# tirtho109/parallel_AMG

Measured on AMD Instinct MI355X. Metric: V-cycle iters/sec + fine-SpMV HBM GB/s, 3D Poisson 128M dofs at 1/2/4/8 GPU, higher is better.
Workload: dtype f64; 1 GPU; poisson3d 512^3 fp64, SA-AMG V(1,1) weighted-Jacobi, 1 part(s); n=134217728, nnz_fine=937951232, levels=6, max_coarse=1000, parallelism=row-slab partition p1

## Files before the change

parallel_amg_amd/_lib.py:

```python
from __future__ import annotations

import contextlib
import ctypes as C
import os

_HERE = os.path.dirname(os.path.abspath(__file__))
LIB_PATH = os.environ.get("PAMG_LIB") or os.path.join(_HERE, "libpamg.so")

PAMG_OK = 0
ERRORS = {-1: "PAMG_E_ARG", -2: "PAMG_E_HIP", -3: "PAMG_E_RCCL", -4: "PAMG_E_OVERFLOW",
          -5: "PAMG_E_SETUP", -6: "PAMG_E_STATE", -7: "PAMG_E_NOMEM"}


class PamgError(RuntimeError):
    def __init__(self, code, fn, msg):
        super().__init__(f"{fn} -> {ERRORS.get(code, code)}: {msg}")
        self.code = code


vp = C.c_void_p
i32, i64, dbl = C.c_int, C.c_int64, C.c_double
pvp = C.POINTER(C.c_void_p)
pi64 = C.POINTER(C.c_int64)
pdbl = C.POINTER(C.c_double)
# ... 95 lines not shown
}
_RESTYPE = {"pamg_version": C.c_char_p, "pamg_last_error": C.c_char_p}

_lib = None


def lib():
    global _lib
    if _lib is None:
        if not os.path.exists(LIB_PATH):
            raise ImportError(
                f"{LIB_PATH} is missing: build it with `python -c 'import __graft_entry__ as g; g.build()'` "
                "(or `make -C parallel_amg_amd/csrc`). There is no CPU fallback.")
        L = C.CDLL(LIB_PATH)
        for name, args in SIGNATURES.items():
            f = getattr(L, name)
            f.argtypes = args
            f.restype = _RESTYPE.get(name, C.c_int)
        _lib = L
    return _lib


class _DlInfo(C.Structure):
    _fields_ = [("dli_fname", C.c_char_p), ("dli_fbase", C.c_void_p),
                ("dli_sname", C.c_char_p), ("dli_saddr", C.c_void_p)]


def runtime_providers() -> dict:
    L = lib()
    dl = C.CDLL(None)
    dladdr = dl.dladdr
    dladdr.argtypes = [C.c_void_p, C.POINTER(_DlInfo)]
    out = {}
    for key, sym in (("hip", "hipStreamCreateWithFlags"), ("rccl", "ncclCommInitRank")):
        try:
            addr = C.cast(getattr(L, sym), C.c_void_p).value
        except AttributeError:
            continue
        info = _DlInfo()
        if addr and dladdr(addr, C.byref(info)) and info.dli_fname:
            out[key] = os.path.realpath(info.dli_fname.decode())
    return out


def call(name, *args):
    L = lib()
    rc = getattr(L, name)(*args)
    if rc != PAMG_OK:
        msg = L.pamg_last_error().decode(errors="replace")
        raise PamgError(rc, name, msg)
    return rc


@contextlib.contextmanager
def option(key: str, value: int):
    old = C.c_int64()
    call("pamg_get_option", key.encode(), C.byref(old))
    call("pamg_set_option", key.encode(), int(value))
    try:
        yield
    finally:
        call("pamg_set_option", key.encode(), old.value)


def layout_of(M, part_set: int = 0) -> dict:
    out = (C.c_int * 10)()
    call("pamg_mat_layout", M.handle, part_set, out)
    win = (C.c_int * 16)()
    if part_set == 0:
        call("pamg_mat_ell_window", M.handle, win)
    return {"ell_xwin": bool(win[0]), "ell_xwin_groups": int(win[1]), "ell_gather_groups": int(win[2]),
            "ell_xwin_max_window": int(win[3]), "ell_xwin_noncontig_groups": int(win[4]),
            "ell_xwin_max_pairs": int(win[5]), "ell_xwin_max_chunks": int(win[6]),
            "ell_xwin_census": {"groups": int(win[7]), "full_groups": int(win[13]), "window_mean": int(win[8]),
                                "window_p95": int(win[9]), "runs_mean": int(win[10]), "runs_max": int(win[11]),
                                "pairs_mean": int(win[12])},
            "c24": bool(out[0]), "vd": bool(out[1]), "rl8": bool(out[2]), "cd": int(out[3]),
            "cd_offsets": int(out[4]), "tm": bool(out[5]), "tm_rs": int(out[6]),
            "tile_nnz": int(out[7]), "tiles": int(out[8]), "anchored": bool(out[9] & 1), "per_tile": bool(out[9] & 2),
            "x_stage": bool(out[9] & 4), "sym": bool(out[9] & 8), "sym_rows": 2 if out[9] & 16 else 1,
            "jr_fused": bool(out[9] & 32), "tm_vd": bool(out[9] & 64), "sym_vd": bool(out[9] & 128),
            "ell": bool(out[9] & 512), "pnc": bool(out[9] & 1024),
            "rpat": bool(out[9] & 2048), "pnc_compact": bool(out[9] & 4096),
            "ell_pair": bool(out[9] & 8192)}


def last_error() -> str:
    return lib().pamg_last_error().decode(errors="replace")


def ptr(a):
    return C.c_void_p(a.ctypes.data) if a is not None and a.size else None
```

parallel_amg_amd/csrc/kernels.hip:

```cpp

#include "pamg_device.h"
#include "div_rn.h"

namespace pamg {
namespace {

__device__ __forceinline__ int wave_incl_scan(int v) {
    const int lane = threadIdx.x & 63, rl = lane & 15;
    int t;
    t = __builtin_amdgcn_mov_dpp(v, 0x111, 0xf, 0xf, false);
    if (rl >= 1) v += t;
    t = __builtin_amdgcn_mov_dpp(v, 0x112, 0xf, 0xf, false);
    if (rl >= 2) v += t;
    t = __builtin_amdgcn_mov_dpp(v, 0x114, 0xf, 0xf, false);
    if (rl >= 4) v += t;
    t = __builtin_amdgcn_mov_dpp(v, 0x118, 0xf, 0xf, false);
    if (rl >= 8) v += t;
    t = __builtin_amdgcn_mov_dpp(v, 0x142, 0xf, 0xf, false);
    if (lane & 16) v += t;
    t = __builtin_amdgcn_mov_dpp(v, 0x143, 0xf, 0xf, false);
    if (lane >= 32) v += t;
    return v;
}

// ... 1786 lines not shown
#pragma unroll
    for (int q = 0; q < NS; ++q) {
        zs[q] = zc0 + q * part;
        ze[q] = min(zc1, zs[q] + part);
        zl[q] = ze[q] > zs[q] ? ze[q] - 1 : zc1 - 1;
    }
    PncRow cur[NS];
    int am[NS], ap[NS];
#pragma unroll
    for (int q = 0; q < NS; ++q) {
        const int z = min(zs[q], zl[q]);
        pnc_load<OP, CP>(cur[q], z * M + ixy, nrows, nx, anc, rec, cid, x, b, y);
        am[q] = anc[z > 0 ? (z - 1) * M + ixy : ixy];
        ap[q] = anc[z + 1 < nz ? (z + 1) * M + ixy : ixy];
    }
    __syncthreads();
    for (int j = 0; j < part; ++j) {
        int zq[NS], L[NS], col[NS][kPncMaxLen];
        double xv[NS][kPncMaxLen];
#pragma unroll
        for (int q = 0; q < NS; ++q) {
            zq[q] = min(zs[q] + j, zl[q]);
            const uint32_t pid = CP ? cur[q].rec.x : cur[q].rec.x & 1023u;
            const uint32_t pw = pid < (uint32_t)npat ? lp[pid] : 0u;
            L[q] = (int)(pw & 7u);
#pragma unroll
            for (int k = 0; k < kPncMaxLen; ++k) {
                const uint32_t c = (pw >> (3 + 3 * k)) & 7u;
                const int c01 = c & 1u ? cur[q].an[1] : cur[q].an[0];
                const int c23 = c & 1u ? cur[q].an[3] : cur[q].an[2];
                const int c45 = c & 1u ? am[q] : cur[q].an[4];
                const int c03 = c & 2u ? c23 : c01;
                const int c47 = c & 2u ? ap[q] : c45;
                col[q][k] = c & 4u ? c47 : c03;
                xv[q][k] = x[k < L[q] ? col[q][k] : col[q][0]];
            }
        }
        PncRow nxt[NS];
        int ap2[NS];
#pragma unroll
        for (int q = 0; q < NS; ++q) {
            const int zn = min(zq[q] + 1, zl[q]);
            pnc_load<OP, CP>(nxt[q], zn * M + ixy, nrows, nx, anc, rec, cid, x, b, y);
            ap2[q] = anc[zn + 1 < nz ? (zn + 1) * M + ixy : zn * M + ixy];
        }
#pragma unroll
        for (int q = 0; q < NS; ++q) {
            const int i = zq[q] * M + ixy;
            uint64_t rr;
            if constexpr (CP) rr = cur[q].rec.x < (uint32_t)npat ? lw[cur[q].rec.x] : 0ull;
            else rr = (((uint64_t)cur[q].rec.y << 32) | cur[q].rec.x) >> 10;
            double s = 0.0, dg = 0.0;
#pragma unroll
            for (int k = 0; k < kPncMaxLen; ++k) {
                const bool ok = k < L[q];
                const double v = lv[(uint32_t)(rr >> (7 * k)) & 127u];
                const double p = v * xv[q][k];
                const double t = s + p;
                s = ok ? t : s;
                if constexpr (OP == OP_JACOBI) dg = ok && col[q][k] == i ? v : dg;
            }
            double out;
            if constexpr (OP == OP_SPMV) {
                out = s;
            } else if constexpr (OP == OP_RESID) {
                out = cur[q].p0 - s;
            } else if constexpr (OP == OP_JACOBI) {
                const double uu = cur[q].p0 - s;
                const double v = omega * uu;
                const double w = v / dg;
                out = cur[q].p1 + w;
            } else {
                out = cur[q].p0 + s;
            }
            const bool in = CP ? cur[q].rec.x != (uint32_t)kPncCombSkip : (cur[q].rec.x & 1023u) != (uint32_t)kPncSkip;
            if (zs[q] + j < ze[q] && in) y[i] = out;
            am[q] = cur[q].an[0];
            cur[q] = nxt[q];
            ap[q] = ap2[q];
        }
    }
}

template <int OP>
__global__ __launch_bounds__(kBlock) void k_rows_long(
    const int* __restrict__ rows, const int* __restrict__ rowptr, const int* __restrict__ col,
    const double* __restrict__ val, const double* __restrict__ x, const double* __restrict__ b,
    double* __restrict__ y, double omega, double c1 = 0.0, const double* __restrict__ xold = nullptr) {
    __shared__ double lprod[kBlock + 8];
    __shared__ double ldiag;
    const int tid = threadIdx.x;
    const int r = rows[blockIdx.x];
    const int z0 = rowptr[r], z1 = rowptr[r + 1];
    double s = 0.0;
    for (int base = z0; base < z1; base += kBlock) {
        const int k = base + tid;
        double p = 0.0;
        if (k < z1) {
            const int c = col[k];
            const double v = val[k];
            p = v * x[c];
            if constexpr (kDiagOp<OP>) {
                if (c == r) ldiag = v;
            }
        }
        lprod[tid] = p;
        __syncthreads();
        if (tid == 0) s = row_sum_lds(lprod, 0, min(kBlock, z1 - base), s);
        __syncthreads();
    }
    if constexpr (OP == OP_CHEB) {
        if (tid == 0) epilogue<OP>(r, s, x, b, y, omega, ldiag, c1, xold);
    } else {
        if (tid == 0) epilogue<OP>(r, s, x, b, y, omega, OP == OP_JACOBI ? ldiag : 0.0);
    }
}

__global__ __launch_bounds__(kBlock) void k_cheb_update(int64_t n, const uint8_t* __restrict__ mask, int mask_bytes,
                                                        const uint8_t* __restrict__ ids,
                                                        const uint32_t* __restrict__ mtab, uint32_t in_flag,
                                                        const double* __restrict__ diag, const double* __restrict__ x,
                                                        const double* __restrict__ xold, double* __restrict__ y,
                                                        double c1, double c2) {
    for (int64_t i = blockIdx.x * (int64_t)kBlock + threadIdx.x; i < n; i += (int64_t)gridDim.x * kBlock) {
        const uint32_t m = ids ? mtab[ids[i]]
                               : (mask_bytes == 1 ? (uint32_t)mask[i] : (uint32_t)reinterpret_cast<const uint16_t*>(mask)[i]);
        if (!(m & in_flag)) continue;
        y[i] = cheb_step(y[i], x[i], xold ? xold[i] : 0.0, diag[i], c1, c2);
    }
}

__global__ void k_jacobi_zero(int64_t n, const double* __restrict__ b,
                              const double* __restrict__ diag, double omega,
                              double* __restrict__ y) {
    for (int64_t i = blockIdx.x * (int64_t)blockDim.x + threadIdx.x; i < n;
         i += (int64_t)gridDim.x * blockDim.x) {
        const double u = b[i] - 0.0;
        const double v = omega * u;
        const double w = v / diag[i];
        y[i] = 0.0 + w;
    }
}

constexpr int kGemvChunk = 1024;
__global__ __launch_bounds__(kBlock) void k_dense_gemv(int64_t n_rows, int64_t n,
                                                       int64_t row0,
                                                       const double* __restrict__ ainv,
                                                       const double* __restrict__ b,
                                                       double* __restrict__ y) {
    __shared__ __attribute__((aligned(16))) double lp_all[kBlock / 64][kGemvChunk + 8];
    const int w = threadIdx.x >> 6, lane = threadIdx.x & 63;
    const int64_t i = (int64_t)blockIdx.x * (kBlock / 64) + w;
    if (i >= n_rows) return;
    const double* a = ainv + (row0 + i) * n;
    double* lp = lp_all[w];
    double s = 0.0;
    for (int64_t c = 0; c < n; c += kGemvChunk) {
        const int m = (int)((n - c) < kGemvChunk ? (n - c) : kGemvChunk);
#pragma unroll
        for (int q = 0; q < kGemvChunk / 64; ++q) {
            const int j = lane + 64 * q;
            if (j < m) {
                const double p = a[c + j] * b[c + j];
                lp[j] = p;
            }
        }
// ... 226 lines not shown
          (int64_t)sd.nbands * sd.band >= A.nrows && A.nrows == (int64_t)sd.tb.nx * sd.tb.ny * sd.tb.nz &&
          A.nrows % 2 == 0))
        return false;
    TbGeom g = sd.tb;
    const int tiles = g.tiles_x * g.tiles_y;
    int zc = options().zm_chunks > 0 ? options().zm_chunks : std::min((1024 + tiles - 1) / tiles, g.nz / 16);
    zc = std::max(1, std::min(zc, g.nz));
    g.zlen = (g.nz + zc - 1) / zc;
    g.zchunks = (g.nz + g.zlen - 1) / g.zlen;
    const int gr = (tiles * g.zchunks + 7) / 8 * 8;
    k_sym_zm<OP><<<gr, kZmThreads, 0, s>>>((int)A.nrows, sd.d_tid, sd.d_vtab, sd.d_mtab, sd.vd_n, g, x, b, y, omega,
                                           ch.c1, ch.xold);
    return true;
}

template <int OP, int NU>
void launch_sym_nu(const pamg_mat& A, const double* x, const double* b, double* y, double omega, hipStream_t s) {
    const SymDia& sd = A.sym;
    const int grid = sd.nbands * 8 * sd.eighth;
    if constexpr (NU == 3) {
        if (launch_sym_zm<OP>(A, x, b, y, omega, s)) return;
    }
    if (sd.vd_n) {
        const int ch = NU <= 3 ? options().symd_chunks : 1;
        const int g = 8 * ((sd.nbands * sd.eighth + ch - 1) / ch);
        if constexpr (NU <= 3) {
            if (ch == 2) {
                k_rows_symd<OP, NU, 2><<<g, kBlock, 0, s>>>((int)A.nrows, (int)A.nrows, sd.d_tid, sd.d_vtab,
                                                            sd.d_mtab, sd.vd_n, sd, x, b, y, omega);
                return;
            }
            if (ch == 4) {
                k_rows_symd<OP, NU, 4><<<g, kBlock, 0, s>>>((int)A.nrows, (int)A.nrows, sd.d_tid, sd.d_vtab,
                                                            sd.d_mtab, sd.vd_n, sd, x, b, y, omega);
                return;
            }
        }
        k_rows_symd<OP, NU><<<grid, kBlock, 0, s>>>((int)A.nrows, (int)A.nrows, sd.d_tid, sd.d_vtab, sd.d_mtab,
                                                  sd.vd_n, sd, x, b, y, omega);
        return;
    }
    if (sd.rpl == 2) {
        k_rows_sym2<OP, NU><<<grid, kBlock, 0, s>>>((int)A.nrows, (int)A.nrows, sd.d_mask, sd.d_diag, sd.d_upper,
                                                  sd.ld, sd, x, b, y, omega);
        return;
    }
    k_rows_sym<OP, NU><<<grid, kBlock, 0, s>>>((int)A.nrows, (int)A.nrows, sd.d_mask, sd.d_diag, sd.d_upper, sd.ld,
                                             sd, x, b, y, omega);
}

template <int OP>
void launch_sym(const pamg_mat& A, const double* x, const double* b, double* y, double omega, hipStream_t s,
                Cheb ch = Cheb{}) {
    if constexpr (OP == OP_PROLONG) {
        return;
    } else if constexpr (OP == OP_CHEB) {
        if (launch_sym_zm<OP_CHEB>(A, x, b, y, omega, s, ch)) return;
        launch_sym<OP_RESID>(A, x, b, y, 0.0, s);
        launch_cheb_update(A, x, ch.xold, y, ch.c1, omega, s);
    } else {
        switch (A.sym.nu) {
            case 1: launch_sym_nu<OP, 1>(A, x, b, y, omega, s); break;
            case 2: launch_sym_nu<OP, 2>(A, x, b, y, omega, s); break;
            case 3: launch_sym_nu<OP, 3>(A, x, b, y, omega, s); break;
            case 4: launch_sym_nu<OP, 4>(A, x, b, y, omega, s); break;
            case 5: launch_sym_nu<OP, 5>(A, x, b, y, omega, s); break;
            case 6: launch_sym_nu<OP, 6>(A, x, b, y, omega, s); break;
            default: launch_sym_nu<OP, 7>(A, x, b, y, omega, s); break;
        }
    }
}

constexpr int kPncZlen = 32, kPncStreams = 2;

template <int OP>
void launch_pnc(const pamg_mat& A, const double* x, const double* b, double* y, double omega, hipStream_t s) {
    const PncSet& P = A.pnc;
    const int zlen = std::min(kPncZlen, P.nz);
    const int nxb = P.nx * P.ny / 256, units = nxb * ((P.nz + zlen - 1) / zlen);
    auto go = [&](auto kern) {
        kern<<<(units + 7) / 8 * 8, 256, 0, s>>>((int)A.nrows, P.nx, P.nx * P.ny, P.nz, zlen, P.d_anc, P.d_rec, P.d_cid,
                                                P.d_pvals, P.d_ptab, P.npat, P.d_vtab, P.nval, x, b, y, omega);
    };
    if (P.d_cid) go(k_rows_pnc<OP, kPncStreams, true>);
    else go(k_rows_pnc<OP, kPncStreams, false>);
}

template <int OP>
void launch_rpat(const pamg_mat& A, const double* x, const double* b, double* y, double omega, hipStream_t s) {
    const RpatSet& R = A.rpat;
    const int grid = (int)((R.ngroups + 7) / 8 * 8);
    auto go = [&](auto kern) {
        kern<<<grid, kEllGroup, 0, s>>>((int)A.nrows, R.d_gorder, R.d_anc, R.d_pid, R.d_pmeta, R.npat, R.d_pent, R.nent,
                                        R.d_vtab, R.nval, (int)R.ngroups, x, b, y, omega);
    };
    go(k_rows_rpat<OP, 8>);
}

template <int OP>
void launch_rows_op(const pamg_mat& A, const TileSet& ts, const double* x, const double* b,
                    double* y, double omega, hipStream_t s, Cheb ch = Cheb{}) {
    if (ts.sym) launch_sym<OP>(A, x, b, y, omega, s, ch);
    if (ts.ell) {
        const EllSet& E = A.ell;
        const int grid = (int)((E.ngroups + 7) / 8 * 8);
        auto go = [&](auto kern) {
            kern<<<grid, kEllGroup, 0, s>>>((int)A.nrows, E.d_gorder, E.d_anc, E.d_smeta, E.d_ci, E.d_vi, E.d_len,
                                            E.d_gmeta, E.d_otab, E.d_vtab, (int)E.ngroups, x, b, y, omega, ch.c1,
                                            ch.xold);
        };
        if (E.win) {
            const int win = std::max(E.max_window, 128);
            const size_t lds = sizeof(double) * (size_t)(win + 256) + sizeof(uint16_t) * 4 * 256;
            k_rows_ellw<OP><<<grid, kEllGroup, lds, s>>>(
                (int)A.nrows, E.d_gslices, E.d_smeta, E.d_ci, E.d_len, E.d_dpos, E.d_gmeta, E.d_otab, E.d_vtab, E.d_wmeta,
                E.d_chunks, E.d_lof, win, (reinterpret_cast<uintptr_t>(x) & 15) != 0 ? 1 : 0, (int)E.ngroups, x, b, y,
                omega, ch.c1, ch.xold);
        } else if (E.d_anc) {
            if (E.paired) go(k_rows_ell<OP, true, true>);
            else go(k_rows_ell<OP, true, false>);
        } else {
            if (E.paired) go(k_rows_ell<OP, false, true>);
            else go(k_rows_ell<OP, false, false>);
        }
    }
    if constexpr (OP != OP_CHEB) {
        if (ts.pnc) launch_pnc<OP>(A, x, b, y, omega, s);
        if (ts.rpat) launch_rpat<OP>(A, x, b, y, omega, s);
    }
    if (ts.n_short > 0) {
        if (ts.tile_nnz == 1024) launch_tile<OP, 1024>(A, ts, x, b, y, omega, s, ch);
        else if (ts.tile_nnz == 4096) launch_tile<OP, 4096>(A, ts, x, b, y, omega, s, ch);
        else launch_tile<OP, 2048>(A, ts, x, b, y, omega, s, ch);
    }
    if (ts.n_long > 0)
        k_rows_long<OP><<<ts.n_long, kBlock, 0, s>>>(ts.d_long, A.d_rowptr, A.d_col, A.d_val, x,
                                                     b, y, omega, ch.c1, ch.xold);
}
}

void launch_sym_tb(const pamg_mat& A, const TbArgs& ta, hipStream_t s) {
    SymDia sd = A.sym;
    TbGeom& g = sd.tb;
    g.zlo = sd.part_lo == 0 ? 0 : sd.part_lo + ta.nstages - 1;
    g.zhi = sd.part_hi == g.nz ? g.nz : sd.part_hi - (ta.nstages - 1);
    const int span = g.zhi - g.zlo;
    if (span <= 0) return;
    g.zchunks = std::max(1, std::min(g.zchunks, span / 2 > 0 ? span / 2 : 1));
    g.zlen = (span + g.zchunks - 1) / g.zchunks;
    g.zchunks = (span + g.zlen - 1) / g.zlen;
    const int ntiles = g.tiles_x * g.tiles_y * g.zchunks;
    const int grid = (ntiles + 7) / 8 * 8;
    g.xfast = options().tb_xfast;
    if (sd.vd_n) {
        if (ta.nstages == 2)
            k_sym_zc<2, 2><<<grid, ZcShape<2>::threads, 0, s>>>((int)A.nrows, sd.d_tid, sd.d_vtab, sd.d_mtab, sd.vd_n,
                                                                sd, ta);
        else
            k_sym_zc<3, 1><<<grid, ZcShape<3>::threads, 0, s>>>((int)A.nrows, sd.d_tid, sd.d_vtab, sd.d_mtab, sd.vd_n,
                                                                sd, ta);
        return;
    }
    if (ta.nstages == 2)
        k_sym_tb<2><<<grid, TbShape<2>::threads, 0, s>>>((int)A.nrows, sd.d_mask, sd.d_diag, sd.d_upper, sd.ld, sd, ta);
    else
        k_sym_tb<3><<<grid, TbShape<3>::threads, 0, s>>>((int)A.nrows, sd.d_mask, sd.d_diag, sd.d_upper, sd.ld, sd, ta);
}

// ... 91 lines not shown
```

parallel_amg_amd/csrc/pamg_device.h:

```cpp
#pragma once

#include <hip/hip_runtime.h>
#include <rccl/rccl.h>

#include <atomic>
#include <cstdint>
#include <array>
#include <mutex>
#include <vector>

#include "pamg_common.h"

namespace pamg {

constexpr int kBlock = 256;
constexpr int kTileRows = 256;

constexpr int kXsMaxClusters = 12;
constexpr int kTmSmallTab = 128;
constexpr int kXsCap = 1088;
constexpr int kXsIoff = 128;
constexpr int kXsGap = 48;
struct XStage {
    int ncl = 0, stride = 0, zix = -1, ncols = 0;
// ... 51 lines not shown
    int tile_order = 1;
    int col24 = 1;
    int long_tiles = 1;
    int long_tiles_min = 24;
    int row_len8 = 1;
    int value_dict = 1;
    int col_dict = 1;
    int tile_major = 1;
    int col_dict_tile = 1;
    int tm_tile_dicts = 1;
    int band_pct = 100;
    int band_pct_restrict = 50;
    int x_stage = 1;
    int col_dict_anchor = 1;
    int poison_ghosts = 0;
    int sym_dia = 1;
    int sym_rows = 2;
    int jr_fuse = 1;
    int symd_chunks = 2;
    int chain_store_x = 0;
    int tb_xfast = 1;
    int sym_zm = 1;
    int zm_chunks = 0;
    int ell = 1;
    int ell_min_rows = 65536;
    int ell_restrict = 1;
    int ell_yblock = 16;
    int rpat = 1;
    int ell_pair = 1;
    int ell_xwin = 1;
    int ell_xwin_max = 7168;
    int pnc_compact = 1;
    int pnc = 1;
    int sym_vd = 1;
};

constexpr int kSymMaxU = 7;
constexpr int kSymVdMax = 64;
struct TbGeom {
    int nx = 0, ny = 0, nz = 0;
    int tiles_x = 0, tiles_y = 0;
    int zchunks = 1, zlen = 0;
    int zlo = 0, zhi = 0;
    int xfast = 0;
};
constexpr int kEllW = 64;
constexpr int kEllGroup = 256;
constexpr int kEllSkip = 255;
constexpr int kEllWinCap = 7168;
constexpr int kEllWinChunks = 256;
constexpr int kEllLdsPerCu = 160 * 1024;
constexpr int kEllWinKeep = 85;
constexpr int kEllWinMinShare = 50;
constexpr int kEllWinMinRatio100 = 150;
struct EllSet {
    int64_t nslices = 0, ngroups = 0;
    int2* d_smeta = nullptr;
    uint32_t* d_ci = nullptr;
    uint32_t* d_vi = nullptr;
    uint8_t* d_len = nullptr;
    int4* d_gmeta = nullptr;
    int* d_otab = nullptr;
    double* d_vtab = nullptr;
    int* d_anc = nullptr;
    int* d_gorder = nullptr;
    int64_t words = 0, otab_n = 0, vtab_n = 0;
    bool paired = false;
    bool win = false;
    int4* d_gslices = nullptr;
    int4* d_wmeta = nullptr;
    int2* d_chunks = nullptr;
    uint16_t* d_lof = nullptr;
    uint8_t* d_dpos = nullptr;
    int64_t nchunks = 0, lof_n = 0;
    int win_groups = 0, gather_groups = 0, noncontig_groups = 0;
    int max_window = 0, max_pairs = 0, max_chunks = 0;
    int mean_window = 0, p95_window = 0, mean_runs = 0, max_runs = 0, mean_pairs = 0, full_groups = 0;
};

constexpr int kPncPatMax = 1024, kPncValMax = 128, kPncMaxLen = 7;
constexpr int kPncSkip = kPncPatMax - 1;
constexpr int kPncCombMax = 1024;
constexpr int kPncCombSkip = 0xffff;
struct PncSet {
    int nx = 0, ny = 0, nz = 0;
    int* d_anc = nullptr;
    uint2* d_rec = nullptr;
    uint16_t* d_cid = nullptr;
    uint64_t* d_pvals = nullptr;
    uint32_t* d_ptab = nullptr;
    double* d_vtab = nullptr;
    int npat = 0, nval = 0;
    int grid = 0;
};

constexpr int kRpatMax = 255, kRpatEnt = 4096, kRpatMaxLen = 128;
constexpr int kRpatSkip = 255;
struct RpatSet {
    int64_t ngroups = 0;
    int* d_anc = nullptr;
    uint8_t* d_pid = nullptr;
    int2* d_pmeta = nullptr;
    uint32_t* d_pent = nullptr;
    double* d_vtab = nullptr;
    int* d_gorder = nullptr;
    int npat = 0, nent = 0, nval = 0;
};

struct SymDia {
    int nu = 0;
    int off[kSymMaxU] = {};
    int64_t ld = 0;
    int band = 0, band_blocks = 0, eighth = 0, nbands = 0;
    int rpl = 1;
    bool tb_ok = false;
    bool tb_part = false;
    int part_lo = 0, part_hi = 0;
    int plane0 = 0;
    int gap_at = 1 << 30, gap = 0;
    TbGeom tb;
    uint8_t* d_mask = nullptr;
    int mask_bytes = 2;
    double* d_diag = nullptr;
    double* d_upper = nullptr;
    int vd_n = 0;
    int vd_main = 0;
    uint8_t* d_tid = nullptr;
    double* d_vtab = nullptr;
    uint32_t* d_mtab = nullptr;
};
Options& options();

}

struct pamg_ctx {
    int device = 0;
    std::atomic<int> refs{1};
    hipStream_t s_comp = nullptr;
    hipStream_t s_comm = nullptr;
    hipEvent_t ev_fork = nullptr, ev_join = nullptr;
    ncclComm_t comm = nullptr;
    int rank = 0, nranks = 1;
    pamg_host_comm_fn host_fn = nullptr;
    void* host_user = nullptr;
    pamg_world* world = nullptr;
    hipEvent_t ev_ready = nullptr;
    std::vector<double> h_send, h_recv;
    double* d_red = nullptr;
    int red_cap = 0;
    double* h_red = nullptr;
    char* stage[2] = {nullptr, nullptr};
    hipEvent_t stage_done[2] = {nullptr, nullptr};
    std::vector<std::array<int64_t, 4>> grids;
    std::mutex grids_mu;
};

void ctx_ref(pamg_ctx* ctx);
void ctx_unref(pamg_ctx* ctx);

struct pamg_plan {
    pamg_ctx* ctx = nullptr;
    int64_t n_own = 0, n_ghost = 0;
    std::vector<int> nbr;
    std::vector<int64_t> recv_off, send_off;
    int* d_send_idx = nullptr;
    double* d_sendbuf = nullptr;
// ... 70 lines not shown
```

parallel_amg_amd/csrc/runtime.hip:

```cpp
#include <dlfcn.h>

#include <algorithm>
#include <array>
#include <atomic>
#include <functional>
#include <iterator>
#include <chrono>
#include <cmath>
#include <condition_variable>
#include <mutex>
#include <cstdio>
#include <cstdlib>
#include <cstring>
#include <map>
#include <memory>
#include <mutex>
#include <string>
#include <thread>
#include <vector>

#include "pamg_device.h"

using pamg::fail;

// ... 2068 lines not shown
        (n_own_cols == nrows || pamg::options().ell_restrict)) {
        CHECK(build_ell(A, u.rp, u.ci, u.val, n_own_cols != nrows, u.inner));
        if (A->interior.ell) u.inner.clear();
        u.tr.mark("ell");
    }
    return PAMG_OK;
}

int64_t ell_bytes(const pamg_mat* A) {
    if (!A->interior.ell) return 0;
    const int64_t nrows = A->nrows;
    return (A->ell.paired ? 4 : 8) * A->ell.words + nrows + 8 * A->ell.nslices + 16 * A->ell.ngroups + 4 * A->ell.otab_n +
           8 * A->ell.vtab_n + (A->ell.d_anc ? 4 * nrows : 0) +
           (A->ell.win ? 32 * A->ell.ngroups + 8 * A->ell.nchunks + 2 * A->ell.lof_n + nrows : 0);
}

void ell_report(const pamg_mat* A, const pamg::TileSet& t, int out[10]) {
    if (!t.ell) return;
    out[8] = (int)A->ell.ngroups;
    out[9] |= 512 | (A->ell.paired ? 8192 : 0);
}

void ell_window(const pamg_mat* A, int out[16]) {
    const pamg::EllSet& E = A->ell;
    const bool w = A->interior.ell && E.win;
    out[0] = w ? 1 : 0;
    out[1] = w ? E.win_groups : 0;
    out[2] = w ? E.gather_groups : 0;
    out[3] = w ? E.max_window : 0;
    out[4] = w ? E.noncontig_groups : 0;
    out[5] = w ? E.max_pairs : 0;
    out[6] = w ? E.max_chunks : 0;
    out[7] = w ? (int)E.ngroups : 0;
    out[8] = w ? E.mean_window : 0;
    out[9] = w ? E.p95_window : 0;
    out[10] = w ? E.mean_runs : 0;
    out[11] = w ? E.max_runs : 0;
    out[12] = w ? E.mean_pairs : 0;
    out[13] = w ? E.full_groups : 0;
    out[14] = out[15] = 0;
}

void ell_free(pamg::EllSet& E) {
    dfree(E.d_gorder);
    dfree(E.d_smeta);
    dfree(E.d_ci);
    dfree(E.d_vi);
    dfree(E.d_len);
    dfree(E.d_gmeta);
    dfree(E.d_otab);
    dfree(E.d_vtab);
    dfree(E.d_anc);
    dfree(E.d_gslices);
    dfree(E.d_wmeta);
    dfree(E.d_chunks);
    dfree(E.d_lof);
    dfree(E.d_dpos);
    E = pamg::EllSet{};
}

int pnc_try(Upload& u) {
    pamg_mat* A = u.A;
    const int64_t nrows = A->nrows;
    if (pamg::options().pnc && u.n_own_cols < nrows && (int64_t)u.inner.size() * 4 >= (int64_t)nrows * 3) {
        const auto grids = grids_of(A->ctx);
        for (auto g = grids.rbegin(); g != grids.rend() && !A->interior.pnc; ++g)
            if ((*g)[0] == nrows) CHECK(build_pnc(A, u.rp, u.ci, u.val, *g, u.inner));
        if (A->interior.pnc) u.inner.clear();
        u.tr.mark("pnc");
    }
    return PAMG_OK;
}

int64_t pnc_bytes(const pamg_mat* A) {
    if (!A->interior.pnc) return 0;
    return (A->pnc.d_cid ? 6 : 12) * A->nrows + (A->pnc.d_cid ? 12 : 4) * A->pnc.npat + 8 * A->pnc.nval;
}

void pnc_report(const pamg_mat* A, const pamg::TileSet& t, int out[10]) {
    if (!t.pnc) return;
    out[3] = A->pnc.nval;
    out[4] = A->pnc.npat;
    out[8] = A->pnc.grid;
    out[9] |= 1024 | (A->pnc.d_cid ? 4096 : 0);
}

void pnc_free(pamg::PncSet& P) {
    dfree(P.d_anc);
    dfree(P.d_rec);
    dfree(P.d_cid);
    dfree(P.d_pvals);
    dfree(P.d_ptab);
    dfree(P.d_vtab);
    P = pamg::PncSet{};
}

int tiles_try(Upload& u) {
    pamg_mat* A = u.A;
    pamg_ctx* ctx = A->ctx;
    const PtrVec& rp = u.rp;
    const IdxVec& ci = u.ci;
    const int64_t nrows = A->nrows, nnz = A->nnz, n_own_cols = u.n_own_cols;
    std::vector<uint16_t> lo;
    std::vector<uint8_t> hi, vidx;
    {
        std::vector<int4> t_in, t_bd;
        const bool square = n_own_cols == nrows;
        const bool tall = n_own_cols < nrows;
        const int64_t tb = u.inner.empty() && u.bnd.empty() ? 0 : u.band();
        CHECK(build_tiles(rp, u.inner, square, &A->interior, tb, ci, &lo, &hi, u.val, &vidx, &t_in, tall));
        CHECK(build_tiles(rp, u.bnd, square, &A->boundary, tb, ci, &lo, &hi, u.val, &vidx, &t_bd, tall));
        u.tr.mark("tiles");
        std::vector<uint8_t> idx8;
        CHECK(build_col_dicts(A, rp, ci, t_in, t_bd, &idx8));
        u.tr.mark("col dicts");
        CHECK(build_tile_major(A, n_own_cols, rp, ci, u.val, t_in, t_bd, lo, hi, idx8));
        u.tr.mark("tile-major");
    }
    if (A->interior.rl8 || A->boundary.rl8) {
        std::vector<uint8_t> rl(nrows + kVecPad, 0);
        par_for(nrows, [&](int64_t a, int64_t b) {
            for (int64_t i = a; i < b; ++i) rl[i] = (uint8_t)std::min<int64_t>(255, rp[i + 1] - rp[i]);
        });
        CHECK(dalloc(&A->d_rlen, nrows + kVecPad));
        CHECK(h2d(ctx, A->d_rlen, rl.data(), rl.size()));
    }
    if (!vidx.empty()) {
        CHECK(dalloc(&A->d_vidx, (int64_t)vidx.size()));
        CHECK(h2d(ctx, A->d_vidx, vidx.data(), vidx.size()));
    }
    if (!lo.empty()) {
        lo.resize(nnz + kVecPad, 0);
        hi.resize(nnz + kVecPad, 0);
        CHECK(dalloc(&A->d_clo, nnz + kVecPad));
        CHECK(dalloc(&A->d_chi, nnz + kVecPad));
        CHECK(h2d(ctx, A->d_clo, lo.data(), sizeof(uint16_t) * lo.size()));
        CHECK(h2d(ctx, A->d_chi, hi.data(), sizeof(uint8_t) * hi.size()));
    }
    u.tr.mark("rest");
    return PAMG_OK;
}

int64_t tiles_bytes(const pamg_mat* A) {
    int64_t sum = 0;
    for (const pamg::TileSet* t : {&A->interior, &A->boundary}) {
        if (t->sym || t->ell || t->pnc || t->rpat) continue;
        const int64_t ns = t->n_short, nz = t->nnz_short;
        int64_t b = 8 * (int64_t)t->n_long + 12 * t->nnz_long;
        const bool base = t->c24 && !t->cd;
        if (t->tm) {
            const int64_t tn = t->tile_nnz;
            const int64_t rowb = t->tm_rs;
            const int64_t valb = t->tm_vt ? tn + 8 * (int64_t)t->tm_vt : 8 * tn;
            b += ns * (rowb * (t->anc ? 5 : 1) + valb + (t->cd ? t->cd * tn / 8 : 3 * tn) + 16 + (base ? 4 : 0)) +
                 (t->cd ? 4 * t->ctab_n * (t->pt ? ns : 1) : 0);
        } else {
            b += (t->rl8 ? 1 : 4) * t->rows_short;
            b += t->cd ? (t->cd * nz + 7) / 8 + 4 * t->ctab_n * (t->pt ? ns : 1) : (t->c24 ? 3 : 4) * nz;
            if (t->pt && t->anc) b += 2 * t->rows_short + 4 * ns;
            b += t->vd ? nz / 2 + 128 * ns : 8 * nz;
            b += (16 + (base ? 4 : 0)) * ns;
        }
        sum += b;
    }
    return sum;
}

// ... 2090 lines not shown
        CHECK(dalloc(&H->pcg_p, cap));
        CHECK(dalloc(&H->pcg_q, cap));
        for (double* p : {H->pcg_r, H->pcg_z, H->pcg_p, H->pcg_q})
            CHECK(dzero(ctx, p, sizeof(double) * cap));
    }
    hipStream_t s = ctx->s_comp;
    double *r = H->pcg_r, *z = H->pcg_z, *p = H->pcg_p, *q = H->pcg_q;
    DeviceSpace d(H, x, b, true);
    double* xd = d.x;
    CHECK(apply(ctx, A, pamg::OP_RESID, xd, d.b, r, 0.0));
    double rr = 0.0;
    CHECK(reduce_scalar(ctx, n, r, r, &rr));
    const double nr0 = std::sqrt(rr);
    if (res_hist) res_hist[0] = nr0;
    int k = 0;
    if (nr0 > 0.0 && maxit > 0) {
        CHECK(vcycle_raw(H, z, r, 1, true));
        HIPC(hipMemcpyAsync(p, z, sizeof(double) * n, hipMemcpyDeviceToDevice, s));
        double rz = 0.0;
        CHECK(reduce_scalar(ctx, n, r, z, &rz));
        while (k < maxit) {
            ++k;
            CHECK(apply(ctx, A, pamg::OP_SPMV, p, nullptr, q, 0.0));
            double pq = 0.0;
            CHECK(reduce_scalar(ctx, n, p, q, &pq));
            const double alpha = rz / pq;
            CHECK(reduce_with(ctx, n, &rr, [&](int np, double* parts, double* res, hipStream_t st) {
                pamg::launch_cg_update(n, alpha, p, q, xd, r, parts, np, res, st);
            }));
            const double nr = std::sqrt(rr);
            if (res_hist) res_hist[k] = nr;
            if (nr <= rtol * nr0) break;
            CHECK(vcycle_raw(H, z, r, 1, true));
            double rz_new = 0.0;
            CHECK(reduce_scalar(ctx, n, r, z, &rz_new));
            const double beta = rz_new / rz;
            rz = rz_new;
            pamg::launch_axpby(n, 1.0, z, beta, p, s);
        }
    }
    d.finish(x);
    HIPC(hipGetLastError());
    HIPC(hipStreamSynchronize(s));
    if (iters) *iters = k;
    return PAMG_OK;
}

}

namespace {
struct OptionRow {
    const char* key;
    int pamg::Options::*member;
    int64_t lo, hi;
    bool pow2;
};
using O = pamg::Options;
const OptionRow kOptionTable[] = {
    {"tile_nnz", &O::tile_nnz, 1024, 4096, true},
    {"tile_order", &O::tile_order, 0, 1, false},
    {"poison_ghosts", &O::poison_ghosts, 0, 1, false},
    {"col24", &O::col24, 0, 1, false},
    {"long_tiles", &O::long_tiles, 0, 1, false},
    {"row_len8", &O::row_len8, 0, 1, false},
    {"value_dict", &O::value_dict, 0, 2, false},
    {"col_dict", &O::col_dict, 0, 1, false},
    {"tile_major", &O::tile_major, 0, 2, false},
    {"col_dict_anchor", &O::col_dict_anchor, 0, 1, false},
    {"col_dict_tile", &O::col_dict_tile, 0, 1, false},
    {"x_stage", &O::x_stage, 0, 1, false},
    {"band_pct", &O::band_pct, 1, 10000, false},
    {"band_pct_restrict", &O::band_pct_restrict, 1, 10000, false},
    {"long_tiles_min", &O::long_tiles_min, 1, 255, false},
    {"tm_tile_dicts", &O::tm_tile_dicts, 0, 1, false},
    {"sym_dia", &O::sym_dia, 0, 1, false},
    {"sym_rows", &O::sym_rows, 1, 2, false},
    {"jr_fuse", &O::jr_fuse, 0, 1, false},
    {"sym_vd", &O::sym_vd, 0, 1, false},
    {"symd_chunks", &O::symd_chunks, 1, 4, true},
    {"sym_zm", &O::sym_zm, 0, 1, false},
    {"tb_xfast", &O::tb_xfast, 0, 1, false},
    {"ell", &O::ell, 0, 1, false},
    {"ell_restrict", &O::ell_restrict, 0, 1, false},
    {"pnc", &O::pnc, 0, 1, false},
    {"rpat", &O::rpat, 0, 1, false},
    {"pnc_compact", &O::pnc_compact, 0, 1, false},
    {"ell_pair", &O::ell_pair, 0, 1, false},
    {"ell_xwin", &O::ell_xwin, 0, 1, false},
    {"ell_xwin_max", &O::ell_xwin_max, 2, pamg::kEllWinCap, false},
    {"ell_yblock", &O::ell_yblock, 0, 65536, false},
    {"ell_min_rows", &O::ell_min_rows, 0, INT32_MAX, false},
    {"zm_chunks", &O::zm_chunks, 0, 4096, false},
    {"chain_store_x", &O::chain_store_x, 0, 1, false},
};

const OptionRow* find_option(const char* key) {
    for (const OptionRow& r : kOptionTable)
        if (std::strcmp(r.key, key) == 0) return &r;
    return nullptr;
}
}

extern "C" {

int pamg_set_option(const char* key, int64_t value) {
    if (!key) return fail(PAMG_E_ARG, "set_option: NULL key");
    const OptionRow* r = find_option(key);
    if (!r || value < r->lo || value > r->hi || (r->pow2 && (value & (value - 1)) != 0))
        return fail(PAMG_E_ARG, "set_option: unknown key or bad value: %s=%lld", key, (long long)value);
    pamg::options().*(r->member) = (int)value;
    return PAMG_OK;
}

int pamg_get_option(const char* key, int64_t* value) {
    if (!key || !value) return fail(PAMG_E_ARG, "get_option: bad args");
    const OptionRow* r = find_option(key);
    if (!r) return fail(PAMG_E_ARG, "get_option: unknown key %s", key);
    *value = pamg::options().*(r->member);
    return PAMG_OK;
}

int pamg_hier_bench_chain(pamg_hier* H, pamg_vec* x, const pamg_vec* b, int reps, double* avg_ms) {
    if (!H || !x || !b || reps < 1 || !avg_ms) return fail(PAMG_E_ARG, "hier_bench_chain: bad args");
    if (!pipe_ok(H, 2, false)) return fail(PAMG_E_STATE, "hier_bench_chain: the hierarchy does not run the cross-cycle pipeline");
    pamg_ctx* ctx = H->ctx;
    CHECK(check_vec_for(H->A[0], x, "hier_bench_chain"));
    CHECK(set_device(ctx));
    CHECK(ensure_u0(H));
    int k = -1;
    return time_reps(ctx->s_comp, reps, avg_ms, [&]() {
        const bool back = k > 0 && (k & 1);
        ++k;
        return launch_chain3(H, x->d, b->d, back ? H->u0 : H->t[0], back ? H->t[0] : H->u0);
    });
}

int pamg_bench_rowop(pamg_ctx* ctx, const pamg_mat* A, int op, pamg_vec* x, const pamg_vec* b,
                     pamg_vec* y, double omega, int reps, double* avg_ms) {
    if (!ctx || !A || !x || !y || reps < 1 || !avg_ms || op < 0 || op > 6)
        return fail(PAMG_E_ARG, "bench_rowop: bad args");
    if ((op == pamg::OP_RESID || op == pamg::OP_JACOBI || op >= 4) && !b) return fail(PAMG_E_ARG, "bench_rowop: b needed");
    if ((op == pamg::OP_JACOBI || op >= 4) && !A->d_diag)
        return fail(PAMG_E_SETUP, "bench_rowop: jacobi needs a square matrix");
    if (op == pamg::OP_CHEB) {
        if (A->interior.pnc || A->interior.rpat) return fail(PAMG_E_ARG, "bench_rowop: op 6 needs a square operator");
        if (x == y || b == y) return fail(PAMG_E_ARG, "bench_rowop: y must differ from x and b");
        CHECK(check_vec_for(A, x, "bench_rowop"));
        if (b->n_own != A->nrows || y->n_own != A->nrows) return fail(PAMG_E_ARG, "bench_rowop: size mismatch");
        CHECK(set_device(ctx));
        double* xo = nullptr;
        CHECK(dalloc(&xo, A->nrows + kVecPad));
        int rc = dzero(ctx, xo, sizeof(double) * (size_t)(A->nrows + kVecPad));
        hipStream_t s = ctx->s_comp;
        if (rc == PAMG_OK)
            rc = time_reps(s, reps, avg_ms, [&]() {
                pamg::launch_rows(*A, A->interior, op, x->d, b->d, xo, y->d, omega, s, omega);
                pamg::launch_rows(*A, A->boundary, op, x->d, b->d, xo, y->d, omega, s, omega);
                return PAMG_OK;
            });
        dfree(xo);
        return rc;
    }
    if (op >= 4 && !(A->interior.sym && (A->sym.tb_ok || A->sym.tb_part)))
        return fail(PAMG_E_STATE, "bench_rowop: op %d needs the temporally blocked layout (pamg_mat_layout bit 5)", op);
    if (op == pamg::OP_PROLONG && (A->interior.sym || A->boundary.sym))
        return fail(PAMG_E_STATE, "bench_rowop: the symmetric layouts have no prolongate-add kernel");
    if (x == y) return fail(PAMG_E_ARG, "bench_rowop: x and y must differ");
// ... 42 lines not shown
```

Measured before the change: 225.2 V-cycles/s.

## Add 2D-tiled pattern-compressed row kernel sharing anchor indices through LDS

Adds a new pattern-compressed (pnc) row kernel that processes a 64x4 xy tile per block and marches along z. Each lane's anchor column indices for its x/y neighbours come from a double-buffered LDS plane with a halo ring, and z-neighbour anchors are carried in registers. This replaces per-row anchor reads from global memory with shared reuse. It is selected when the pnc option is 1 and the grid dims divide the tile, and the option range is widened to 2 so the old kernel stays reachable. The cost is extra LDS, one block barrier per z step, and higher register pressure.

```diff
diff --git a/parallel_amg_amd/_lib.py b/parallel_amg_amd/_lib.py
--- a/parallel_amg_amd/_lib.py
+++ b/parallel_amg_amd/_lib.py
@@ -201,7 +201,7 @@
             "jr_fused": bool(out[9] & 32), "tm_vd": bool(out[9] & 64), "sym_vd": bool(out[9] & 128),
             "ell": bool(out[9] & 512), "pnc": bool(out[9] & 1024),
             "rpat": bool(out[9] & 2048), "pnc_compact": bool(out[9] & 4096),
-            "ell_pair": bool(out[9] & 8192)}
+            "ell_pair": bool(out[9] & 8192), "pnc_tiled": bool(out[9] & 16384)}
 
 
 def last_error() -> str:
diff --git a/parallel_amg_amd/csrc/kernels.hip b/parallel_amg_amd/csrc/kernels.hip
--- a/parallel_amg_amd/csrc/kernels.hip
+++ b/parallel_amg_amd/csrc/kernels.hip
@@ -1892,6 +1892,196 @@
     }
 }
 
+struct PnctRow {
+    uint2 rec;
+    double p0, p1;
+    int am, a0, ap;
+    int rg;
+};
+
+template <int OP, int NS, bool CP, int TX, int TY>
+__global__ __launch_bounds__(256) void k_rows_pnct(int nrows, int nx, int M, int nz, int zlen,
+                                                   const int* __restrict__ anc, const uint2* __restrict__ rec,
+                                                   const uint16_t* __restrict__ cid, const uint64_t* __restrict__ pvals,
+                                                   const uint32_t* __restrict__ ptab, int npat,
+                                                   const double* __restrict__ vtab, int nval,
+                                                   const double* __restrict__ x, const double* __restrict__ b,
+                                                   double* __restrict__ y, double omega) {
+    static_assert(TX * TY == 256 && 2 * TX + 2 * TY <= 256, "one row per lane; one ring point per edge thread");
+    constexpr int LW = TX + 2, LP = LW * (TY + 2);
+    __shared__ uint32_t lp[CP ? kPncCombMax : kPncPatMax];
+    __shared__ uint64_t lw[CP ? kPncCombMax : 1];
+    __shared__ double lv[kPncValMax];
+    __shared__ int la[NS][2][LP];
+    const int nxb = M >> 8;
+    const int units = nxb * ((nz + zlen - 1) / zlen);
+    const int per = (units + 7) >> 3;
+    const int u = (int)(blockIdx.x & 7) * per + (int)(blockIdx.x >> 3);
+    if (u >= units) return;
+    const int tid = (int)threadIdx.x;
+    for (int t = tid; t < npat; t += 256) lp[t] = ptab[t];
+    if constexpr (CP)
+        for (int t = tid; t < npat; t += 256) lw[t] = pvals[t];
+    for (int t = tid; t < nval; t += 256) lv[t] = vtab[t];
+    const int zc0 = (u / nxb) * zlen, zc1 = min(nz, zc0 + zlen);
+    const int part = (zc1 - zc0 + NS - 1) / NS;
+    const int tpx = nx / TX, ny = M / nx, tb = u % nxb;
+    const int x0 = (tb % tpx) * TX, y0 = (tb / tpx) * TY;
+    const int ixy = (y0 + tid / TX) * nx + x0 + tid % TX;
+    const int lpos = (tid / TX + 1) * LW + tid % TX + 1;
+    int rxy = -1, rpos = 0;
+    if (tid < TX) {
+        rxy = (y0 > 0 ? y0 - 1 : y0) * nx + x0 + tid;
+        rpos = tid + 1;
+    } else if (tid < 2 * TX) {
+        rxy = (y0 + TY < ny ? y0 + TY : y0 + TY - 1) * nx + x0 + tid - TX;
+        rpos = (TY + 1) * LW + tid - TX + 1;
+    } else if (tid >= 256 - TY) {
+        rxy = (y0 + tid - (256 - TY)) * nx + (x0 + TX < nx ? x0 + TX : x0 + TX - 1);
+        rpos = (tid - (256 - TY) + 1) * LW + TX + 1;
+    } else if (tid >= 256 - 2 * TY) {
+        rxy = (y0 + tid - (256 - 2 * TY)) * nx + (x0 > 0 ? x0 - 1 : x0);
+        rpos = (tid - (256 - 2 * TY) + 1) * LW;
+    }
+    int zs[NS], ze[NS], zl[NS], za[NS];
+    PnctRow r[NS];
+#pragma unroll
+    for (int q = 0; q < NS; ++q) {
+        zs[q] = zc0 + q * part;
+        ze[q] = min(zc1, zs[q] + part);
+        zl[q] = ze[q] > zs[q] ? ze[q] - 1 : zc1 - 1;
+        const int z = za[q] = min(zs[q], zl[q]), zp = min(z + 1, nz - 1), i = z * M + ixy;
+        if constexpr (CP) r[q].rec = make_uint2((uint32_t)cid[i], 0u);
+        else r[q].rec = rec[i];
+        r[q].p0 = 0.0;
+        r[q].p1 = 0.0;
+        if constexpr (OP == OP_RESID || OP == OP_JACOBI) r[q].p0 = b[i];
+        if constexpr (OP == OP_PROLONG) r[q].p0 = y[i];
+        if constexpr (OP == OP_JACOBI) r[q].p1 = x[i];
+        r[q].a0 = anc[i];
+        r[q].am = anc[z > 0 ? i - M : i];
+        r[q].ap = anc[zp * M + ixy];
+        r[q].rg = 0;
+        la[q][0][lpos] = r[q].a0;
+        if (rxy >= 0) {
+            la[q][0][rpos] = anc[z * M + rxy];
+            r[q].rg = anc[zp * M + rxy];
+        }
+    }
+    __syncthreads();
+    for (int j = 0; j < part; ++j) {
+        uint32_t pw[NS];
+        int an[NS][4], lmax = 0;
+#pragma unroll
+        for (int q = 0; q < NS; ++q) {
+            const uint32_t pid = CP ? r[q].rec.x : r[q].rec.x & 1023u;
+            pw[q] = pid < (uint32_t)npat ? lp[pid] : 0u;
+            lmax = max(lmax, (int)(pw[q] & 7u));
+            const int* pl = &la[q][j & 1][lpos];
+            an[q][0] = pl[-1];
+            an[q][1] = pl[1];
+            an[q][2] = pl[-LW];
+            an[q][3] = pl[LW];
+            la[q][(j & 1) ^ 1][lpos] = r[q].ap;
+            if (rxy >= 0) la[q][(j & 1) ^ 1][rpos] = r[q].rg;
+        }
+        int col[NS][kPncMaxLen];
+        double xv[NS][kPncMaxLen];
+        uint2 nrec[NS];
+        double np0[NS], np1[NS];
+        int ap2[NS], rg2[NS];
+#pragma unroll
+        for (int q = 0; q < NS; ++q)
+#pragma unroll
+            for (int k = 0; k < kPncMaxLen; ++k) {
+                col[q][k] = -1;
+                xv[q][k] = 0.0;
+            }
+        auto loads = [&](auto lmc) {
+            constexpr int LM = decltype(lmc)::value;
+#pragma unroll
+            for (int q = 0; q < NS; ++q) {
+                const int L = (int)(pw[q] & 7u);
+#pragma unroll
+                for (int k = 0; k < LM; ++k) {
+                    const uint32_t c = (pw[q] >> (3 + 3 * k)) & 7u;
+                    const int c01 = c & 1u ? an[q][0] : r[q].a0;
+                    const int c23 = c & 1u ? an[q][2] : an[q][1];
+                    const int c45 = c & 1u ? r[q].am : an[q][3];
+                    const int c03 = c & 2u ? c23 : c01;
+                    const int c47 = c & 2u ? r[q].ap : c45;
+                    col[q][k] = c & 4u ? c47 : c03;
+                    xv[q][k] = x[k < L ? col[q][k] : col[q][0]];
+                }
+            }
+        };
+        const int lm = 3 + (__any(lmax > 3) ? 1 : 0) + (__any(lmax > 4) ? 1 : 0) + (__any(lmax > 5) ? 1 : 0) +
+                       (__any(lmax > 6) ? 1 : 0);
+        switch (lm) {
+            case 3: loads(std::integral_constant<int, 3>{}); break;
+            case 4: loads(std::integral_constant<int, 4>{}); break;
+            case 5: loads(std::integral_constant<int, 5>{}); break;
+            case 6: loads(std::integral_constant<int, 6>{}); break;
+            default: loads(std::integral_constant<int, 7>{}); break;
+        }
+#pragma unroll
+        for (int q = 0; q < NS; ++q) {
+            const int in = min(zs[q] + j + 1, zl[q]) * M + ixy, z2 = min(za[q] + 2, nz - 1);
+            if constexpr (CP) nrec[q] = make_uint2((uint32_t)cid[in], 0u);
+            else nrec[q] = rec[in];
+            np0[q] = 0.0;
+            np1[q] = 0.0;
+            if constexpr (OP == OP_RESID || OP == OP_JACOBI) np0[q] = b[in];
+            if constexpr (OP == OP_PROLONG) np0[q] = y[in];
+            if constexpr (OP == OP_JACOBI) np1[q] = x[in];
+            ap2[q] = anc[z2 * M + ixy];
+            rg2[q] = 0;
+            if (rxy >= 0) rg2[q] = anc[z2 * M + rxy];
+        }
+#pragma unroll
+        for (int q = 0; q < NS; ++q) {
+            const int i = min(zs[q] + j, zl[q]) * M + ixy, L = (int)(pw[q] & 7u);
+            uint64_t rr;
+            if constexpr (CP) rr = r[q].rec.x < (uint32_t)npat ? lw[r[q].rec.x] : 0ull;
+            else rr = (((uint64_t)r[q].rec.y << 32) | r[q].rec.x) >> 10;
+            double s = 0.0, dg = 0.0;
+#pragma unroll
+            for (int k = 0; k < kPncMaxLen; ++k) {
+                const bool ok = k < L;
+                const double v = lv[(uint32_t)(rr >> (7 * k)) & 127u];
+                const double p = v * xv[q][k];
+                const double t = s + p;
+                s = ok ? t : s;
+                if constexpr (OP == OP_JACOBI) dg = ok && col[q][k] == i ? v : dg;
+            }
+            double out;
+            if constexpr (OP == OP_SPMV) {
+                out = s;
+            } else if constexpr (OP == OP_RESID) {
+                out = r[q].p0 - s;
+            } else if constexpr (OP == OP_JACOBI) {
+                const double uu = r[q].p0 - s;
+                const double v = omega * uu;
+                const double w = v / dg;
+                out = r[q].p1 + w;
+            } else {
+                out = r[q].p0 + s;
+            }
+            const bool in = CP ? r[q].rec.x != (uint32_t)kPncCombSkip : (r[q].rec.x & 1023u) != (uint32_t)kPncSkip;
+            if (zs[q] + j < ze[q] && in) y[i] = out;
+            r[q].rec = nrec[q];
+            r[q].p0 = np0[q];
+            r[q].p1 = np1[q];
+            r[q].am = r[q].a0;
+            r[q].a0 = r[q].ap;
+            r[q].ap = ap2[q];
+            r[q].rg = rg2[q];
+            za[q] = min(za[q] + 1, nz - 1);
+        }
+        __syncthreads();
+    }
+}
+
 template <int OP>
 __global__ __launch_bounds__(kBlock) void k_rows_long(
     const int* __restrict__ rows, const int* __restrict__ rowptr, const int* __restrict__ col,
@@ -2284,8 +2474,13 @@
         kern<<<(units + 7) / 8 * 8, 256, 0, s>>>((int)A.nrows, P.nx, P.nx * P.ny, P.nz, zlen, P.d_anc, P.d_rec, P.d_cid,
                                                 P.d_pvals, P.d_ptab, P.npat, P.d_vtab, P.nval, x, b, y, omega);
     };
-    if (P.d_cid) go(k_rows_pnc<OP, kPncStreams, true>);
-    else go(k_rows_pnc<OP, kPncStreams, false>);
+    if (options().pnc == 1 && pnc_tiled(P.nx, P.ny)) {
+        if (P.d_cid) go(k_rows_pnct<OP, kPncStreams, true, kPncTx, kPncTy>);
+        else go(k_rows_pnct<OP, kPncStreams, false, kPncTx, kPncTy>);
+    } else {
+        if (P.d_cid) go(k_rows_pnc<OP, kPncStreams, true>);
+        else go(k_rows_pnc<OP, kPncStreams, false>);
+    }
 }
 
 template <int OP>
diff --git a/parallel_amg_amd/csrc/pamg_device.h b/parallel_amg_amd/csrc/pamg_device.h
--- a/parallel_amg_amd/csrc/pamg_device.h
+++ b/parallel_amg_amd/csrc/pamg_device.h
@@ -157,6 +157,8 @@
 constexpr int kPncSkip = kPncPatMax - 1;
 constexpr int kPncCombMax = 1024;
 constexpr int kPncCombSkip = 0xffff;
+constexpr int kPncTx = 64, kPncTy = 4;
+constexpr bool pnc_tiled(int nx, int ny) { return nx % kPncTx == 0 && ny % kPncTy == 0; }
 struct PncSet {
     int nx = 0, ny = 0, nz = 0;
     int* d_anc = nullptr;
diff --git a/parallel_amg_amd/csrc/runtime.hip b/parallel_amg_amd/csrc/runtime.hip
--- a/parallel_amg_amd/csrc/runtime.hip
+++ b/parallel_amg_amd/csrc/runtime.hip
@@ -2174,7 +2174,7 @@
     out[3] = A->pnc.nval;
     out[4] = A->pnc.npat;
     out[8] = A->pnc.grid;
-    out[9] |= 1024 | (A->pnc.d_cid ? 4096 : 0);
+    out[9] |= 1024 | (A->pnc.d_cid ? 4096 : 0) | (pamg::pnc_tiled(A->pnc.nx, A->pnc.ny) ? 16384 : 0);
 }
 
 void pnc_free(pamg::PncSet& P) {
@@ -4431,7 +4431,7 @@
     {"tb_xfast", &O::tb_xfast, 0, 1, false},
     {"ell", &O::ell, 0, 1, false},
     {"ell_restrict", &O::ell_restrict, 0, 1, false},
-    {"pnc", &O::pnc, 0, 1, false},
+    {"pnc", &O::pnc, 0, 2, false},
     {"rpat", &O::rpat, 0, 1, false},
     {"pnc_compact", &O::pnc_compact, 0, 1, false},
     {"ell_pair", &O::ell_pair, 0, 1, false},
```

After: 229.8 V-cycles/s, median of 6. 1.02x the previous value.
